# akankshabaranwal/graph-algorithm-image-segmentation-GPGPU

Hardware: NVIDIA B200
Metric: Mpixel/s end-to-end segmentation (1080p, Boruvka-Felzenszwalb, 4-connected) (higher is better)
Workload: dtype f32+u64

## Files before the change

graph-algorithm-image-segmentation-gpgpu_b200/csrc/gseg_api.cu:

```cuda
#include <cuda_runtime.h>
#include <dlfcn.h>
#include <nvjpeg.h>
#include <limits.h>
#include <stddef.h>
#include <math.h>
#include <stdio.h>
#include <stdlib.h>
#include <string.h>

#include <new>
#include <vector>

#include "../../include/gseg.h"
#include "gseg_kernels.cuh"
#include "gseg_sort.cuh"
#include "gseg_dedup.cuh"
#include "gseg_jpeg.hpp"
#include "gseg_jpeg.cuh"

#define GSEG_MAXMARK 1024
#define GRID_CAP (148 * 8)

struct GsegHead {
    GsegRunParams p;
// ... 497 lines not shown
extern "C" int gseg_input_rgb(gseg_ctx *ctx, uint8_t *out, int mem_kind) {
    if (!ctx || !out) return GSEG_E_ARG;
    if (ctx->pending) { const int rc = gseg_wait(ctx); if (rc) return rc; }
    if (!ctx->valid || !ctx->rgb_staged) return fail(ctx, GSEG_E_STATE, "the last run's input was not staged by the context", cudaSuccess);
    if (mem_kind != GSEG_MEM_HOST && mem_kind != GSEG_MEM_DEVICE) return fail(ctx, GSEG_E_ARG, "mem_kind", cudaSuccess);
    CK(cudaSetDevice(ctx->device));
    CK(cudaMemcpyAsync(out, ctx->d_rgb + (size_t)3 * ctx->w * ctx->halo_top, (size_t)3 * ctx->w * ctx->h,
                       mem_kind == GSEG_MEM_HOST ? cudaMemcpyDeviceToHost : cudaMemcpyDeviceToDevice, ctx->stream));
    CK(cudaStreamSynchronize(ctx->stream));
    return GSEG_OK;
}

extern "C" void gseg_destroy(gseg_ctx *ctx) {
    if (!ctx) return;
    cudaSetDevice(ctx->device);
    if (ctx->own_stream) cudaStreamSynchronize(ctx->own_stream);
    cudaFree(ctx->d_rgb); cudaFree(ctx->d_tmp); cudaFree(ctx->d_planes);
    cudaFree(ctx->d_G); cudaFree(ctx->d_wgrid); cudaFree(ctx->d_wsel);
    cudaFree(ctx->d_succ); cudaFree(ctx->d_rank);
    for (int i = 0; i < 2; ++i) {
        cudaFree(ctx->d_best[i]); cudaFree(ctx->d_attr[i]); cudaFree(ctx->d_csum[i]); cudaFree(ctx->d_cmean[i]);
        cudaFree(ctx->d_eab[i]); cudaFree(ctx->d_ew[i]); cudaFree(ctx->d_pcnt[i]); cudaFree(ctx->d_poff[i]); cudaFree(ctx->d_labels[i]);
    }
    cudaFree(ctx->d_pscan); cudaFree(ctx->d_arena); cudaFree(ctx->d_statusC); cudaFree(ctx->d_statusE); cudaFree(ctx->d_ctl);
    jpeg_release(ctx);
    cudaFree(ctx->d_jfile); cudaFree(ctx->d_jsamples); cudaFree(ctx->d_jdev); cudaFree(ctx->d_jcoef);
    if (ctx->h_jdesc) cudaFreeHost(ctx->h_jdesc);
    cudaFree(ctx->d_jerr); cudaFree(ctx->d_jsub);
    if (ctx->ev_jdesc) cudaEventDestroy(ctx->ev_jdesc);
    if (ctx->ev_jdone) cudaEventDestroy(ctx->ev_jdone);
    delete ctx->jplan;
    sort_scratch_free(&ctx->sort);
    cudaFree(ctx->d_xkeys); cudaFree(ctx->d_xvals); cudaFree(ctx->d_xkeep); cudaFree(ctx->d_xab); cudaFree(ctx->d_xw);
    cudaFree(ctx->d_winner); cudaFree(ctx->d_dd);
    for (int i = 0; i <= GSEG_MAXMARK; ++i)
        if (ctx->ev[i]) cudaEventDestroy(ctx->ev[i]);
    if (ctx->h_ctl) cudaFreeHost(ctx->h_ctl);
    if (ctx->h_head) cudaFreeHost(ctx->h_head);
    if (ctx->own_stream) cudaStreamDestroy(ctx->own_stream);
    free(ctx);
}

extern "C" int gseg_set_stream(gseg_ctx *ctx, void *s) {
    if (!ctx) return GSEG_E_ARG;
    if (ctx->pending) return GSEG_E_STATE;
    ctx->stream = s ? (cudaStream_t)s : ctx->own_stream;
    return GSEG_OK;
}

extern "C" int gseg_tail_cluster(const gseg_ctx *ctx) { return ctx ? ctx->tail_cluster : GSEG_E_ARG; }
extern "C" int gseg_tail_cluster_from_env(const gseg_ctx *ctx) { return ctx && ctx->tail_cluster_env ? 1 : 0; }
extern "C" void *gseg_get_stream(const gseg_ctx *ctx) { return ctx ? (void *)ctx->stream : nullptr; }

extern "C" int gseg_set_tail(gseg_ctx *ctx, uint32_t max_edges, uint32_t max_components) {
    if (!ctx) return GSEG_E_ARG;
    if (ctx->pending) return GSEG_E_STATE;
    ctx->tail_E = max_edges; ctx->tail_V = max_components;
    ctx->nbig_hint = -1;
    return GSEG_OK;
}

extern "C" int gseg_set_dedup(gseg_ctx *ctx, int on, uint32_t min_edges, uint32_t min_ratio, uint32_t max_components) {
    if (!ctx) return GSEG_E_ARG;
    if (ctx->pending) return GSEG_E_STATE;
    CK(cudaSetDevice(ctx->device));
    ctx->dd_on = on != 0;
    if (min_edges) ctx->dd_min_edges = min_edges;
    if (min_ratio) ctx->dd_min_ratio = min_ratio;
    if (max_components) ctx->dd_V = max_components;
    ctx->nbig_hint = -1; ctx->dd_skip = false;
    CK(upload_dd(ctx));
    return GSEG_OK;
}

extern "C" int gseg_set_tail_cluster(gseg_ctx *ctx, int ctas) {
    if (!ctx || ctas < 1 || ctas > 16) return GSEG_E_ARG;
    if (ctx->pending) return GSEG_E_STATE;
    CK(cudaSetDevice(ctx->device));
    ctx->tail_cluster = fit_tail_cluster(ctas);
    return GSEG_OK;
}

extern "C" int gseg_set_blocks_per_sm(gseg_ctx *ctx, int blocks) {
    if (!ctx || blocks < 1 || blocks > 8) return GSEG_E_ARG;
    if (ctx->pending) return GSEG_E_STATE;
    ctx->occ_mult = blocks;
    return GSEG_OK;
}

static int gauss_mask(float sigma, float *mask) {
    if (sigma < 0.01f) sigma = 0.01f;
    const int len = (int)ceilf(sigma * 4.0f) + 1;
    if (len > GSEG_MAXMASK) return -1;
    double m[GSEG_MAXMASK], s = 0.0;
    for (int i = 0; i < len; ++i) {
        const double t = (double)i / (double)sigma;
        m[i] = exp(-0.5 * t * t);
    }
    for (int i = 1; i < len; ++i) s += m[i];
    s = 2.0 * s + m[0];
    for (int i = 0; i < len; ++i) mask[i] = (float)(m[i] / s);
    return len;
}

static inline void mark(gseg_ctx *c, cudaStream_t s, const char *name, int round) {
    ++c->launches;
    if (!c->profiling || c->n_marks >= GSEG_MAXMARK) return;
    if (!c->ev[c->n_marks]) cudaEventCreate(&c->ev[c->n_marks]);
    cudaEventRecord(c->ev[c->n_marks], s);
    c->mark_name[c->n_marks] = name;
    c->mark_round[c->n_marks] = round;
    ++c->n_marks;
}
static inline void mark_end(gseg_ctx *c, cudaStream_t s) {
    if (!c->profiling || c->n_marks == 0 || c->n_marks >= GSEG_MAXMARK) return;
    if (!c->ev[c->n_marks]) cudaEventCreate(&c->ev[c->n_marks]);
    cudaEventRecord(c->ev[c->n_marks], s);
    c->mark_name[c->n_marks] = nullptr;
    c->mark_round[c->n_marks] = -1;
    ++c->n_marks;
}

static GsegBufs bufs_of(const gseg_ctx *c) {
    GsegBufs B;
    B.planes = c->d_planes; B.G = c->d_G; B.wgrid = c->d_wgrid;
    B.succ = c->d_succ; B.rank = c->d_rank; B.wsel = c->d_wsel; B.arena = c->d_arena;
    for (int i = 0; i < 2; ++i) {
        B.best[i] = c->d_best[i]; B.attr[i] = c->d_attr[i]; B.csum[i] = c->d_csum[i]; B.cmean[i] = c->d_cmean[i];
        B.eab[i] = c->d_eab[i]; B.ew[i] = c->d_ew[i]; B.pcnt[i] = c->d_pcnt[i]; B.poff[i] = c->d_poff[i];
    }
    B.statusC = c->d_statusC; B.statusE = c->d_statusE; B.pscan = c->d_pscan;
    return B;
}

template <int R>
static size_t blur_smem() { return (size_t)3 * (TH + 2 * R) * (BLUR_PF(R) + BLUR_PH * sizeof(float)); }
template <int R>
static void launch_blur(gseg_ctx *c, cudaStream_t s, int ntiles) {
    static bool attr[64] = {false};
    if (!attr[c->device & 63]) { cudaFuncSetAttribute(k_blur_tile<R>, cudaFuncAttributeMaxDynamicSharedMemorySize, (int)blur_smem<R>()); attr[c->device & 63] = true; }
    k_blur_tile<R><<<ntiles, NT, blur_smem<R>(), s>>>(c->d_ctl, c->d_planes);
}

template <int VARIANT, int D>
static size_t graph_smem() {
    return (size_t)(3 + D + (VARIANT == GSEG_SUPERPIX ? 1 : 0)) * BH * BW * sizeof(float) + 16;
}
template <int VARIANT, int D>
static void launch_r0_graph(gseg_ctx *c, cudaStream_t s, int ntiles, const GsegBufs &B) {
    static bool attr[64] = {false};
    if (!attr[c->device & 63]) { cudaFuncSetAttribute(k_r0_graph<VARIANT, D>, cudaFuncAttributeMaxDynamicSharedMemorySize, (int)graph_smem<VARIANT, D>()); attr[c->device & 63] = true; }
    k_r0_graph<VARIANT, D><<<ntiles < c->num_sms * c->occ_mult ? ntiles : c->num_sms * c->occ_mult, NT, graph_smem<VARIANT, D>(), s>>>(c->d_ctl, B);
}
template <int D, bool SP>
static void launch_r0_edges(gseg_ctx *c, cudaStream_t s, size_t V, const GsegBufs &B) {
    const size_t ntiles = ((size_t)D * ((V + GSEG_PAGE - 1) / GSEG_PAGE) + NT / 32 - 1) / (NT / 32);
    k_r0_edges<D, SP><<<(int)(ntiles < (size_t)c->num_sms * c->occ_mult ? ntiles : (size_t)c->num_sms * c->occ_mult), NT, 0, s>>>(c->d_ctl, B);
}

static void enqueue_round0(gseg_ctx *c, cudaStream_t s) {
    const size_t V = (size_t)c->w * c->h;
    const int variant = c->params.variant, D = c->D;
    const bool sp = variant == GSEG_SUPERPIX;
    const GsegBufs B = bufs_of(c);
    const int ntiles = ((c->w + TW - 1) / TW) * ((c->h + TH - 1) / TH);
    const int ntilesG = ((c->w + TW - 1) / TW) * ((c->h + GH - 1) / GH);
    const int R = c->h_head->p.mask_len - 1;
    if (R >= 1 && R <= 8) {
        mark(c, s, "k_blur_tile", 0);
        switch (R) {
        case 1: launch_blur<1>(c, s, ntiles); break;
        case 2: launch_blur<2>(c, s, ntiles); break;
        case 3: launch_blur<3>(c, s, ntiles); break;
        case 4: launch_blur<4>(c, s, ntiles); break;
        case 5: launch_blur<5>(c, s, ntiles); break;
        case 6: launch_blur<6>(c, s, ntiles); break;
        case 7: launch_blur<7>(c, s, ntiles); break;
        default: launch_blur<8>(c, s, ntiles); break;
        }
    } else {
        mark(c, s, "k_blur_h", 0);
        k_blur_h<<<grid_for((size_t)c->w * c->h_head->p.h_in, NT), NT, 0, s>>>(c->d_ctl, c->d_tmp);
        mark(c, s, "k_blur_v", 0);
        k_blur_v<<<grid_for(3 * V, NT), NT, 0, s>>>(c->d_ctl, c->d_tmp, c->d_planes);
    }
    if (sp) {
        mark(c, s, "k_sobel", 0);
        k_sobel<<<grid_for(V, NT), NT, 0, s>>>(c->d_ctl, c->d_planes, c->d_G);
    }
    mark(c, s, "k_r0_graph", 0);
    if (variant == GSEG_FELZ) { if (D == 2) launch_r0_graph<GSEG_FELZ, 2>(c, s, ntilesG, B); else launch_r0_graph<GSEG_FELZ, 4>(c, s, ntilesG, B); }
    else if (variant == GSEG_HIER) { if (D == 2) launch_r0_graph<GSEG_HIER, 2>(c, s, ntilesG, B); else launch_r0_graph<GSEG_HIER, 4>(c, s, ntilesG, B); }
    else { if (D == 2) launch_r0_graph<GSEG_SUPERPIX, 2>(c, s, ntilesG, B); else launch_r0_graph<GSEG_SUPERPIX, 4>(c, s, ntilesG, B); }
    mark(c, s, "k_relabel", 0);
    if (sp) k_relabel<true, true><<<grid_for(V, NT), NT, 0, s>>>(c->d_ctl, B);
    else k_relabel<true, false><<<grid_for(V, NT), NT, 0, s>>>(c->d_ctl, B);
    if (sp) {
        mark(c, s, "k_means", 0);
        k_means<<<grid_for(V, NT, c->num_sms * c->occ_mult), NT, 0, s>>>(c->d_ctl, B);
    }
    mark(c, s, "k_r0_edges", 0);
    if (D == 2) { if (sp) launch_r0_edges<2, true>(c, s, V, B); else launch_r0_edges<2, false>(c, s, V, B); }
    else { if (sp) launch_r0_edges<4, true>(c, s, V, B); else launch_r0_edges<4, false>(c, s, V, B); }
}

static void enqueue_round(gseg_ctx *c, cudaStream_t s, int r, size_t Vb, size_t Pb) {
    const bool sp = c->params.variant == GSEG_SUPERPIX;
    const GsegBufs B = bufs_of(c);
    const int cap = c->num_sms * c->occ_mult;
    if (Pb > GSEG_PSCAN_INLINE) {
        mark(c, s, "k_page_scan", r);
        k_page_scan<<<grid_for(Pb, 1024, 64), 1024, 0, s>>>(c->d_ctl, B);
    }
    mark(c, s, "k_succ_scan", r);
    if (sp) k_succ_scan<true><<<grid_for(Vb, NT * CPT, cap) + 1, NT, 0, s>>>(c->d_ctl, B);
    else k_succ_scan<false><<<grid_for(Vb, NT * CPT, cap) + 1, NT, 0, s>>>(c->d_ctl, B);
    mark(c, s, "k_relabel", r);
    if (sp) k_relabel<false, true><<<grid_for(Vb, NT, cap), NT, 0, s>>>(c->d_ctl, B);
    else k_relabel<false, false><<<grid_for(Vb, NT, cap), NT, 0, s>>>(c->d_ctl, B);
    if (sp) {
        mark(c, s, "k_means", r);
        k_means<<<grid_for(Vb, NT, cap), NT, 0, s>>>(c->d_ctl, B);
    }
    mark(c, s, "k_edges", r);
    if (sp) k_edges<true><<<grid_for(Pb, NT / 32, cap), NT, 0, s>>>(c->d_ctl, B);
    else k_edges<false><<<grid_for(Pb, NT / 32, cap), NT, 0, s>>>(c->d_ctl, B);
}

static u32 dedup_V(const gseg_ctx *c) {
    const u32 v = c->dd_V > 2u ? c->dd_V : 2u;
    return v < 65536u ? v : 65536u;
}
static bool dedup_enabled(const gseg_ctx *c) {
    return c->dd_on && c->params.variant != GSEG_SUPERPIX && !(c->params.flags & GSEG_FLAG_NO_DEDUP);
}
static bool dedup_enqueue(const gseg_ctx *c) {
    return dedup_enabled(c) &&
           !(c->dd_skip && c->hint_w == c->w && c->hint_h == c->h && c->hint_variant == c->params.variant && c->hint_conn == c->params.connectivity);
}
static void enqueue_dedup(gseg_ctx *c, cudaStream_t s, int round) {
    const GsegBufs B = bufs_of(c);
    const int cap = c->num_sms * c->occ_mult;
    const size_t ntiles = (c->dd_cap + SORT_TILE - 1) / SORT_TILE;
    const int gs = (int)(ntiles < (size_t)c->num_sms * 2 ? ntiles : (size_t)c->num_sms * 2);
    mark(c, s, "k_dd_plan", round);
    k_dd_plan<<<1, 1024, 0, s>>>(c->d_ctl, B, c->d_dd);
    mark(c, s, "k_dd_keys", round);
    k_dd_keys<<<cap, NT, 0, s>>>(c->d_ctl, B, c->d_dd);
    mark(c, s, "k_sort_scan", round);
    k_sort_scan_dev<<<4, SORT_RADIX, 0, s>>>(&c->d_dd->sort);
    for (int p = 0; p < 4; ++p) {
        mark(c, s, "k_sort_onesweep", round);
        k_sort_onesweep_dev<<<gs, SORT_NT, sort_smem_bytes(), s>>>(&c->d_dd->sort, p);
    }
    mark(c, s, "k_dd_select", round);
    k_dd_select<<<cap, NT, 0, s>>>(c->d_dd);
    mark(c, s, "k_dd_mark", round);
    k_dd_mark<<<cap, NT, 0, s>>>(c->d_ctl, B, c->d_dd);
    mark(c, s, "k_dd_compact", round);
    k_dd_compact<<<grid_for(c->dd_cap, 4096, c->num_sms * 2), 1024, 0, s>>>(c->d_ctl, B, c->d_dd);
    mark(c, s, "k_dd_finish", round);
    k_dd_finish<<<cap, NT, 0, s>>>(c->d_ctl, B, c->d_dd);
}
static bool dedup_wanted_host(const gseg_ctx *c) {
    const RoundState &st = c->h_ctl->st;
    return dedup_enabled(c) && st.phase != PH_DONE && st.round >= 1u && st.V >= 2u && st.V <= dedup_V(c) && st.E <= c->dd_cap &&
           st.E >= c->dd_min_edges && st.E / st.V >= c->dd_min_ratio;
}

static cudaError_t enqueue_tail(gseg_ctx *c, cudaStream_t s) {
    cudaLaunchConfig_t cfg = {};
    cudaLaunchAttribute at[1];
    cfg.gridDim = dim3(c->tail_cluster); cfg.blockDim = dim3(NTT);
    cfg.dynamicSmemBytes = TAIL_SMEM; cfg.stream = s;
    at[0].id = cudaLaunchAttributeClusterDimension;
    at[0].val.clusterDim.x = c->tail_cluster; at[0].val.clusterDim.y = 1; at[0].val.clusterDim.z = 1;
    cfg.attrs = at; cfg.numAttrs = 1;
    GsegCtl *ctl = c->d_ctl;
    GsegBufs B = bufs_of(c);
    mark(c, s, "k_tail", -1);
    if (c->params.variant == GSEG_SUPERPIX) return cudaLaunchKernelEx(&cfg, k_tail<true>, ctl, B);
    return cudaLaunchKernelEx(&cfg, k_tail<false>, ctl, B);
}

static size_t edge_slots(const gseg_ctx *ctx) {
    return (size_t)ctx->Dmax * ((ctx->Vmax + GSEG_PAGE - 1) / GSEG_PAGE + 1) * GSEG_PAGE;
}

static int max_rounds_of(const gseg_params *p) {
    int r = p->max_rounds > 0 ? p->max_rounds : 48;
    return r > GSEG_MAXR ? GSEG_MAXR : r;
}

static int readback(gseg_ctx *ctx) {
    CK(cudaMemcpyAsync(ctx->h_ctl, ctx->d_ctl, sizeof(GsegCtl), cudaMemcpyDeviceToHost, ctx->stream));
    CK(cudaStreamSynchronize(ctx->stream));
    return GSEG_OK;
}

static int finish(gseg_ctx *ctx) {
    ctx->pending = false;
    if (ctx->h_ctl->error == DERR_SCAN) return fail(ctx, GSEG_E_INTERNAL, "look-back watchdog", cudaSuccess);
    if (ctx->h_ctl->error == DERR_ARENA) return fail(ctx, GSEG_E_ARENA, "map arena", cudaSuccess);
    if (ctx->h_ctl->error == DERR_CHASE) return fail(ctx, GSEG_E_INTERNAL, "successor cycle", cudaSuccess);
    if (ctx->h_ctl->error == DERR_JPEG) return fail(ctx, GSEG_E_ARG, "corrupt JPEG: the entropy-coded data does not decode", cudaSuccess);
    if (ctx->h_ctl->error >= DERR_CHECK) {
        snprintf(ctx->err, sizeof(ctx->err), "checked build: bounds check at site %u failed", ctx->h_ctl->error - DERR_CHECK);
        return GSEG_E_INTERNAL;
    }
    const GsegCtl *h = ctx->h_ctl;
// ... 880 lines not shown
```

graph-algorithm-image-segmentation-gpgpu_b200/csrc/gseg_kernels.cuh:

```cuda
#pragma once
#include <cooperative_groups.h>

#include "gseg_device.cuh"

namespace cg = cooperative_groups;

#define NT 256
#ifndef GSEG_LB_SUCC
#define GSEG_LB_SUCC 4
#endif
#ifndef GSEG_LB_EDGES
#define GSEG_LB_EDGES 4
#endif
#define NTT 1024
#define CPT 4
#ifndef RUNWIN
#define RUNWIN 4
#endif

#define TW 64
#ifndef TH
#define TH 32
#endif
#define BW (TW + 4)
// ... 407 lines not shown

#define GSEG_PSCAN_INLINE 32768u
#define GSEG_TAIL_STAGE 16384u
__device__ __forceinline__ void block_scan_pages(const u32 *pcnt, u32 P, u32 *pscan, u32 *s) {
    const int lane = threadIdx.x & 31, wid = threadIdx.x >> 5, nwarp = blockDim.x >> 5;
    u32 carry = 0;
    for (u32 base = 0; base < P; base += 16u * blockDim.x) {
        const u32 i = base + 16u * threadIdx.x;
        u32 q[16];
        if (i + 15u < P) {
#pragma unroll
            for (int k = 0; k < 4; ++k) {
                const uint4 t = __ldcg(reinterpret_cast<const uint4 *>(pcnt + i) + k);
                q[4 * k] = t.x; q[4 * k + 1] = t.y; q[4 * k + 2] = t.z; q[4 * k + 3] = t.w;
            }
        } else {
#pragma unroll
            for (int k = 0; k < 16; ++k) q[k] = i + k < P ? __ldcg(pcnt + i + k) : 0u;
        }
        u32 v = 0;
#pragma unroll
        for (int k = 0; k < 16; ++k) { const u32 t = q[k]; q[k] = v; v += t; }
        const u32 inc = warp_incl_scan(v, lane);
        if (lane == 31) s[wid] = inc;
        __syncthreads();
        if (wid == 0) {
            const u32 x = lane < nwarp ? s[lane] : 0u;
            const u32 xi = warp_incl_scan(x, lane);
            s[lane] = xi - x;
            if (lane == 31) s[32] = xi;
        }
        __syncthreads();
        const u32 e = carry + s[wid] + inc - v;
        if (i + 15u < P) {
#pragma unroll
            for (int k = 0; k < 4; ++k)
                reinterpret_cast<uint4 *>(pscan + i)[k] = make_uint4(e + q[4 * k], e + q[4 * k + 1], e + q[4 * k + 2], e + q[4 * k + 3]);
        } else {
#pragma unroll
            for (int k = 0; k < 16; ++k)
                if (i + k < P) pscan[i + k] = e + q[k];
        }
        carry += s[32];
        __syncthreads();
    }
}

template <int NTH, bool R0, bool SP, bool SPREAD = false>
__device__ __forceinline__ void phase_R(const GsegCtl *ctl, const GsegBufs &B, const RoundState &st) {
    constexpr int RPT = (SPREAD || R0) ? 1 : 4;
    const int cur = st.round & 1, nxt = cur ^ 1;
    const u32 V = st.V;
    u32 *map = B.arena + st.map_off;
    const u32 V0 = (u32)ctl->p.w * (u32)ctl->p.h;
    const u32 lane = threadIdx.x & 31u, wid = threadIdx.x >> 5, nwarp = NTH / 32;
    const u32 tile0 = SPREAD ? wid * gridDim.x + blockIdx.x : blockIdx.x * nwarp + wid;
    const u32 ntile = (V + 32u * RPT - 1u) / (32u * RPT);
    for (u32 tile = tile0; tile < ntile; tile += gridDim.x * nwarp) {
        u32 c[RPT], r[RPT];
        bool act[RPT], moved[RPT];
#pragma unroll
        for (int k = 0; k < RPT; ++k) {
            c[k] = (tile * RPT + (u32)k) * 32u + lane;
            act[k] = c[k] < V;
            r[k] = act[k] ? (SPREAD ? ld_relaxed_u32(B.succ + c[k]) : B.succ[c[k]]) : c[k];
            moved[k] = r[k] != c[k];
        }
        bool busy[RPT];
#pragma unroll
        for (int k = 0; k < RPT; ++k) busy[k] = moved[k];
        for (u32 steps = 0;; ++steps) {
            u32 rr[RPT];
            bool any = false;
#pragma unroll
            for (int k = 0; k < RPT; ++k)
                if (busy[k]) rr[k] = SPREAD ? ld_relaxed_u32(B.succ + r[k]) : B.succ[r[k]];
#pragma unroll
            for (int k = 0; k < RPT; ++k)
                if (busy[k]) {
                    if (rr[k] == r[k]) busy[k] = false;
                    else { r[k] = rr[k]; any = true; }
                }
            if (!any) break;
            if (steps > V) { ((GsegCtl *)ctl)->error = DERR_CHASE; break; }
        }
        u32 m[RPT], sz[RPT], iv[RPT];
#pragma unroll
        for (int k = 0; k < RPT; ++k) {
            m[k] = 0u; sz[k] = 1u; iv[k] = 0u;
            if (act[k]) {
                GSEG_CHK(ctl, r[k] < V, 2);
                if (moved[k]) B.succ[c[k]] = r[k];
                m[k] = ld_prev<!SPREAD>(B.rank + r[k]);
                GSEG_CHK(ctl, m[k] < V && (unsigned long long)st.map_off + c[k] < ctl->p.arena_cap, 3);
            }
        }
#pragma unroll
        for (int k = 0; k < RPT; ++k)
            if (act[k]) {
                map[c[k]] = m[k];
                if (!R0) { const uint2 at = ld_prev<!SPREAD>(B.attr[cur] + c[k]); sz[k] = at.x; iv[k] = at.y; }
                if (moved[k]) iv[k] = max(iv[k], __ldcg(B.wsel + c[k]));
            }
#pragma unroll
        for (int k = 0; k < RPT; ++k) {
            warp_run_accumulate(B.attr[nxt], m[k], sz[k], iv[k], act[k]);
            if (SP && act[k]) {
                long long v0, v1, v2;
                const u32 cc = c[k];
                if (R0) { v0 = fx8(B.planes[cc]); v1 = fx8(B.planes[V0 + cc]); v2 = fx8(B.planes[2 * V0 + cc]); }
                else {
                    v0 = __ldcg(B.csum[cur] + 3 * (size_t)cc); v1 = __ldcg(B.csum[cur] + 3 * (size_t)cc + 1);
                    v2 = __ldcg(B.csum[cur] + 3 * (size_t)cc + 2);
                }
                atomicAdd((u64 *)(B.csum[nxt] + 3 * (size_t)m[k]), (u64)v0);
                atomicAdd((u64 *)(B.csum[nxt] + 3 * (size_t)m[k] + 1), (u64)v1);
                atomicAdd((u64 *)(B.csum[nxt] + 3 * (size_t)m[k] + 2), (u64)v2);
            }
        }
    }
}

template <bool SP, bool FILTER>
__device__ __forceinline__ void emit_row(const GsegBufs &B, int nxt, u32 pos, bool act, u32 a, u32 b, u32 wv,
                                         u32 fa = 0xFFFFFFFFu, u32 fb = 0xFFFFFFFFu, u32 *sfilter = nullptr) {
    u32 kb = wv;
    if (act) {
#ifndef GSEG_EXP_NOSTORE
        B.eab[nxt][pos] = make_uint2(a, b);
        B.ew[nxt][pos] = wv;
#endif
        if (SP) kb = __float_as_uint(__fmul_rn(__uint_as_float(wv), mean_dist_m(B.cmean[nxt], a, b)));
    }
#ifndef GSEG_EXP_NOMIN
    warp_run_min2<FILTER, FILTER ? 32 : RUNWIN>(B.best[nxt], a, b, kb, pos, act, fa, fb, sfilter);
#endif
}

template <bool SP>
__device__ __forceinline__ void emit_row_east(const GsegBufs &B, int nxt, u32 pos, bool act, u32 a, u32 b, u32 wv) {
    u32 kb = wv;
    if (act) {
#ifndef GSEG_EXP_NOSTORE
        B.eab[nxt][pos] = make_uint2(a, b);
        B.ew[nxt][pos] = wv;
#endif
        if (SP) kb = __float_as_uint(__fmul_rn(__uint_as_float(wv), mean_dist_m(B.cmean[nxt], a, b)));
    }
#ifndef GSEG_EXP_NOMIN
    warp_chain_min(B.best[nxt], a, b, kb, pos, act, __ballot_sync(0xFFFFFFFFu, act));
#endif
}

template <int D, bool SP>
__global__ void __launch_bounds__(NT, GSEG_LB_EDGES) k_r0_edges(GsegCtl *ctl, GsegBufs B) {
    constexpr int ROWS = GSEG_PAGE / 32;
    const int lane = threadIdx.x & 31;
    const u32 lt = (1u << lane) - 1u;
    const RoundState st = ctl->st;
    const int w = ctl->p.w, h = ctl->p.h;
    const u32 V = (u32)w * (u32)h;
    const u32 *__restrict__ map = B.arena;
    const u32 tpd = (V + GSEG_PAGE - 1) / GSEG_PAGE, ntiles = tpd * (u32)D;
    const u32 nw = gridDim.x * (NT / 32);
    u32 esum = 0;
    if (blockIdx.x == 0 && threadIdx.x == 0) ctl->ticketC = 0;
    for (u32 tile = blockIdx.x * (NT / 32) + (threadIdx.x >> 5); tile < ntiles; tile += nw) {
        const int d = (int)(tile / tpd);
        const int dx = d == 1 ? 0 : 1, dy = d == 0 ? 0 : (d == 3 ? -1 : 1);
        const int off = dy * w + dx;
        const u32 p0 = (tile - (u32)d * tpd) * GSEG_PAGE + lane;
        u32 a[ROWS], b[ROWS], m[ROWS], wv[ROWS];
        const float *wg = B.wgrid + (size_t)d * V + p0;
        int y = (int)(p0 / (u32)w), x = (int)(p0 - (u32)y * (u32)w);
#pragma unroll
        for (int j = 0; j < ROWS; ++j) {
            const u32 p = p0 + 32u * j;
            bool keep = false;
            a[j] = b[j] = wv[j] = 0u;
            if (p < V && x + dx < w && y + dy < h && y + dy >= 0) {
                a[j] = map[p];
                b[j] = map[(u32)((int)p + off)];
                wv[j] = __float_as_uint(wg[32 * j]);
                keep = a[j] != b[j];
            }
            m[j] = __ballot_sync(0xFFFFFFFFu, keep);
            x += 32;
            while (x >= w) { x -= w; ++y; }
        }
        u32 total = 0;
#pragma unroll
        for (int j = 0; j < ROWS; ++j) total += __popc(m[j]);
        if (lane == 0) { B.pcnt[1][tile] = total; B.poff[1][tile] = tile * GSEG_PAGE; }
        GSEG_CHK(ctl, (unsigned long long)tile * GSEG_PAGE + total <= ctl->p.edge_slots, 4);
        esum += total;
        u32 rowoff = tile * GSEG_PAGE;
#pragma unroll
        for (int j = 0; j < ROWS; ++j) {
            if (m[j] == 0u) continue;
            const bool act = (m[j] >> lane) & 1u;
            if (d == 0) emit_row_east<SP>(B, 1, rowoff + __popc(m[j] & lt), act, a[j], b[j], wv[j]);
            else emit_row<SP, false>(B, 1, rowoff + __popc(m[j] & lt), act, a[j], b[j], wv[j]);
            rowoff += __popc(m[j]);
        }
    }
    if (lane == 0 && esum) atomicAdd(&ctl->Eacc[0], esum);
    RoundState s0 = st;
    s0.P = ntiles;
    last_block_advance(ctl, s0, 1u);
}

template <bool SP, bool SPREAD>
__device__ __forceinline__ void phase_S(GsegCtl *ctl, const GsegBufs &B, const RoundState &st, u32 *sh) {
    constexpr u32 TILE_C = 32 * CPT;
    const int lane = threadIdx.x & 31, wid = threadIdx.x >> 5, nwarp = blockDim.x >> 5;
    const u32 lt = (1u << lane) - 1u;
    const int cur = st.round & 1, nxt = cur ^ 1;
    const u32 V = st.V;
    const u32 nwt = (V + TILE_C - 1) / TILE_C;
    const u32 ntiles = (nwt + nwarp - 1) / nwarp;
    const u32 tag = ctl->p.epoch_base + st.round * 2u + 1u;
    const u64 *best = B.best[cur];
    const uint2 *eab = B.eab[cur], *attr = B.attr[cur];
    const float kk = ctl->p.k;
    const u32 min_size = (u32)ctl->p.min_size, phase = st.phase;
    const bool pred = ctl->p.variant == GSEG_FELZ && phase == PH_PRED;
    const bool msz = ctl->p.variant == GSEG_FELZ && phase == PH_MINSIZE;
    if (blockIdx.x == 0 && threadIdx.x == 0) ctl->ticketE = 0;
    u32 stile = (u32)wid * gridDim.x + blockIdx.x;
    auto write_ids = [&](u32 pre, u32 base, const u32 *m, u32 total) {
        u32 rowoff = pre;
#pragma unroll
        for (int j = 0; j < CPT; ++j) {
            if ((m[j] >> lane) & 1u) B.rank[base + 32u * j] = rowoff + __popc(m[j] & lt);
            rowoff += __popc(m[j]);
        }
        for (u32 i = lane; i < total; i += 32u) {
            const u32 n = pre + i;
            B.attr[nxt][n] = make_uint2(0u, 0u); B.best[nxt][n] = GSEG_KEY_NONE;
            if (SP) { B.csum[nxt][3 * (size_t)n] = 0; B.csum[nxt][3 * (size_t)n + 1] = 0; B.csum[nxt][3 * (size_t)n + 2] = 0; }
        }
    };
    auto finish_block = [&](u32 btile, u32 base, u32 below, u32 all, const u32 *m, u32 total) {
        if (wid == 0) {
            const u32 pre = lookback_resolve(B.statusC, btile, tag, all, &ctl->error);
            if (lane == 0) sh[64] = pre;
        }
        __syncthreads();
        const u32 bpre = sh[64];
        if (btile == ntiles - 1 && threadIdx.x == 0) ctl->Vnext = bpre + all;
        write_ids(bpre + below, base, m, total);
        __syncthreads();
    };
    bool p_have = false;
    u32 p_btile = 0, p_base = 0, p_below = 0, p_all = 0, p_total = 0, p_m[CPT] = {};
    for (;;) {
        u32 btile = 0, tile;
        if (SPREAD) {
            tile = stile;
            if (tile >= nwt) break;
            stile += gridDim.x * (u32)nwarp;
        } else {
            if (threadIdx.x == 0) sh[65] = atomicAdd(&ctl->ticketC, 1u);
            __syncthreads();
            btile = sh[65];
            if (btile >= ntiles) break;
            tile = btile * nwarp + wid;
        }
        const u32 base = tile * TILE_C + lane;
        u64 key[CPT], key2[CPT];
        uint2 ab[CPT], ta[CPT], tb[CPT];
#pragma unroll
        for (int j = 0; j < CPT; ++j) key[j] = base + 32u * j < V ? ld_prev<!SPREAD>(best + base + 32u * j) : GSEG_KEY_NONE;
#pragma unroll
        for (int j = 0; j < CPT; ++j) {
            GSEG_CHK(ctl, key[j] == GSEG_KEY_NONE || (u32)key[j] < ctl->p.edge_slots, 5);
            ab[j] = key[j] != GSEG_KEY_NONE ? ld_prev<!SPREAD>(eab + (u32)key[j]) : make_uint2(0u, 0u);
        }
#pragma unroll
        for (int j = 0; j < CPT; ++j) {
            key2[j] = GSEG_KEY_NONE; ta[j] = tb[j] = make_uint2(1u, 0u);
            if (key[j] != GSEG_KEY_NONE) {
                const u32 c = base + 32u * j, other = ab[j].x == c ? ab[j].y : ab[j].x;
                GSEG_CHK(ctl, (ab[j].x == c || ab[j].y == c) && other < V && other != c, 6);
                key2[j] = ld_prev<!SPREAD>(best + other);
                if (pred || msz) { ta[j] = ld_prev<!SPREAD>(attr + ab[j].x); tb[j] = ld_prev<!SPREAD>(attr + ab[j].y); }
            }
        }
        u32 m[CPT], total = 0;
#pragma unroll
        for (int j = 0; j < CPT; ++j) {
            const u32 c = base + 32u * j;
            bool root = false;
            if (c < V) {
                u32 s = c, wb = 0u;
                if (key[j] != GSEG_KEY_NONE) {
                    wb = (u32)(key[j] >> 32);
                    const bool c_is_a = ab[j].x == c;
                    const u32 other = c_is_a ? ab[j].y : ab[j].x;
                    bool ok = true, other_ok = true;
                    if (pred) {
                        const float wt = __uint_as_float(wb);
                        const float fa = __fadd_rn(__uint_as_float(ta[j].y), __fdiv_rn(kk, __uint2float_rn(ta[j].x)));
                        const float fb = __fadd_rn(__uint_as_float(tb[j].y), __fdiv_rn(kk, __uint2float_rn(tb[j].x)));
                        ok = wt <= fa && wt <= fb;
                    } else if (msz) {
                        ok = (c_is_a ? ta[j].x : tb[j].x) < min_size;
                        other_ok = (c_is_a ? tb[j].x : ta[j].x) < min_size;
                    }
                    if (ok) {
                        s = other;
                        if (key2[j] == key[j] && other_ok && c < other) s = c;
                    }
                }
                B.succ[c] = s;
                B.wsel[c] = wb;
                root = s == c;
            }
            m[j] = __ballot_sync(0xFFFFFFFFu, root);
            total += __popc(m[j]);
        }
        if (SPREAD) {
            const u32 pre = lookback_prefix(B.statusC, tile, tag, total, &ctl->error);
            if (tile == nwt - 1 && lane == 0) ctl->Vnext = pre + total;
            write_ids(pre, base, m, total);
        } else {
            if (lane == 0) sh[wid] = total;
            __syncthreads();
            const u32 v = lane < nwarp ? sh[lane] : 0u;
            u32 below = lane < wid ? v : 0u, all = v;
#pragma unroll
            for (int o = 16; o; o >>= 1) { below += __shfl_xor_sync(0xFFFFFFFFu, below, o); all += __shfl_xor_sync(0xFFFFFFFFu, all, o); }
            if (wid == 0) lookback_publish(B.statusC, btile, tag, all);
            __syncthreads();
            if (p_have) finish_block(p_btile, p_base, p_below, p_all, p_m, p_total);
            p_have = true; p_btile = btile; p_base = base; p_below = below; p_all = all; p_total = total;
#pragma unroll
            for (int j = 0; j < CPT; ++j) p_m[j] = m[j];
        }
    }
    if (!SPREAD && p_have) finish_block(p_btile, p_base, p_below, p_all, p_m, p_total);
}

template <bool SP, bool SPREAD, int RW>
__device__ __forceinline__ void phase_E_rows(GsegCtl *ctl, const GsegBufs &B, const RoundState &st, u32 Vnext, u32 *stage) {
    constexpr int ROWS = GSEG_PAGE / 32;
    const int lane = threadIdx.x & 31;
    const u32 lt = (1u << lane) - 1u;
    const int cur = st.round & 1, nxt = cur ^ 1;
    const u32 E = st.E, P = st.P;
    const uint2 *eab = B.eab[cur];
    const u32 *ew = B.ew[cur];
    const u32 *pc = B.pcnt[cur], *po = B.poff[cur];
    const u32 *map = B.arena + st.map_off;
    const bool filter = (E >> ctl->p.filter_shift) > Vnext;
    const u32 G = group_size(st), ngroups = (P + G - 1u) / G;
    if (blockIdx.x == 0 && threadIdx.x == 0) ctl->ticketC = 0;
// ... 458 lines not shown
```

Before: 9685.

## Stage round-0 edge inputs via double-buffered TMA bulk copies per warp

Adds a staged variant of k_r0_edges in which each warp prefetches its next page's label, neighbour-label and weight streams into shared memory with cp.async.bulk and mbarriers, double-buffered, so global loads overlap with compaction and emission of the current page. The host picks the staged variant when pages per warp stay under a threshold and otherwise falls back to the original direct-load path. The staged path needs about 50KB of dynamic shared memory per block, which may lower occupancy, and it adds per-page barrier waits.

Measured after the change: 10060, median of 6. +3.9%, better.

```diff
diff --git a/graph-algorithm-image-segmentation-gpgpu_b200/csrc/gseg_api.cu b/graph-algorithm-image-segmentation-gpgpu_b200/csrc/gseg_api.cu
--- a/graph-algorithm-image-segmentation-gpgpu_b200/csrc/gseg_api.cu
+++ b/graph-algorithm-image-segmentation-gpgpu_b200/csrc/gseg_api.cu
@@ -673,10 +673,16 @@
     if (!attr[c->device & 63]) { cudaFuncSetAttribute(k_r0_graph<VARIANT, D>, cudaFuncAttributeMaxDynamicSharedMemorySize, (int)graph_smem<VARIANT, D>()); attr[c->device & 63] = true; }
     k_r0_graph<VARIANT, D><<<ntiles < c->num_sms * c->occ_mult ? ntiles : c->num_sms * c->occ_mult, NT, graph_smem<VARIANT, D>(), s>>>(c->d_ctl, B);
 }
+#define R0_STAGE_MAX_PPW 128
 template <int D, bool SP>
 static void launch_r0_edges(gseg_ctx *c, cudaStream_t s, size_t V, const GsegBufs &B) {
-    const size_t ntiles = ((size_t)D * ((V + GSEG_PAGE - 1) / GSEG_PAGE) + NT / 32 - 1) / (NT / 32);
-    k_r0_edges<D, SP><<<(int)(ntiles < (size_t)c->num_sms * c->occ_mult ? ntiles : (size_t)c->num_sms * c->occ_mult), NT, 0, s>>>(c->d_ctl, B);
+    static bool attr[64] = {false};
+    if (!attr[c->device & 63]) { cudaFuncSetAttribute(k_r0_edges<D, SP, true>, cudaFuncAttributeMaxDynamicSharedMemorySize, (int)R0_SMEM); attr[c->device & 63] = true; }
+    const size_t pages = (size_t)D * ((V + GSEG_PAGE - 1) / GSEG_PAGE);
+    const size_t ntiles = (pages + NT / 32 - 1) / (NT / 32);
+    const int grid = (int)(ntiles < (size_t)c->num_sms * c->occ_mult ? ntiles : (size_t)c->num_sms * c->occ_mult);
+    if (pages <= (size_t)R0_STAGE_MAX_PPW * grid * (NT / 32)) k_r0_edges<D, SP, true><<<grid, NT, R0_SMEM, s>>>(c->d_ctl, B);
+    else k_r0_edges<D, SP, false><<<grid, NT, 0, s>>>(c->d_ctl, B);
 }
 
 static void enqueue_round0(gseg_ctx *c, cudaStream_t s) {
diff --git a/graph-algorithm-image-segmentation-gpgpu_b200/csrc/gseg_kernels.cuh b/graph-algorithm-image-segmentation-gpgpu_b200/csrc/gseg_kernels.cuh
--- a/graph-algorithm-image-segmentation-gpgpu_b200/csrc/gseg_kernels.cuh
+++ b/graph-algorithm-image-segmentation-gpgpu_b200/csrc/gseg_kernels.cuh
@@ -583,37 +583,144 @@
 #endif
 }
 
-template <int D, bool SP>
+__device__ __forceinline__ u32 smem_addr(const void *p) { return (u32)__cvta_generic_to_shared(p); }
+__device__ __forceinline__ void mbar_init(u64 *bar) {
+    asm volatile("mbarrier.init.shared::cta.b64 [%0], 1;\n\tfence.mbarrier_init.release.cluster;" ::"r"(smem_addr(bar)) : "memory");
+}
+__device__ __forceinline__ void mbar_expect_tx(u64 *bar, u32 bytes) {
+    asm volatile("mbarrier.arrive.expect_tx.shared::cta.b64 _, [%0], %1;" ::"r"(smem_addr(bar)), "r"(bytes) : "memory");
+}
+__device__ __forceinline__ void mbar_wait(u64 *bar, u32 parity) {
+    asm volatile("{\n\t.reg .pred P1;\n\tWAIT:\n\t"
+                 "mbarrier.try_wait.parity.shared::cta.b64 P1, [%0], %1;\n\t"
+                 "@!P1 bra WAIT;\n\t}" ::"r"(smem_addr(bar)), "r"(parity) : "memory");
+}
+__device__ __forceinline__ void bulk_copy(void *dst, const void *src, u32 bytes, u64 *bar) {
+    asm volatile("cp.async.bulk.shared::cluster.global.mbarrier::complete_tx::bytes [%0], [%1], %2, [%3];"
+                 ::"r"(smem_addr(dst)), "l"(src), "r"(bytes), "r"(smem_addr(bar)) : "memory");
+}
+__device__ __forceinline__ void fence_proxy_async() { asm volatile("fence.proxy.async.shared::cta;" ::: "memory"); }
+
+#define R0_STREAM 264
+#define R0_BUF (3 * R0_STREAM)
+#define R0_SMEM ((NT / 32) * (2 * R0_BUF * 4 + 16))
+struct R0Page {
+    int d, off;
+    u32 p0;
+    u32 src[3];
+    u32 n[3];
+};
+__device__ __forceinline__ R0Page r0_page(u32 tile, u32 tpd, u32 V, int w) {
+    R0Page pg;
+    pg.d = (int)(tile / tpd);
+    pg.off = pg.d == 0 ? 1 : pg.d == 1 ? w : pg.d == 2 ? w + 1 : 1 - w;
+    pg.p0 = (tile - (u32)pg.d * tpd) * GSEG_PAGE;
+    const long long end = min((long long)pg.p0 + GSEG_PAGE, (long long)V);
+    const long long lo[3] = {pg.p0, max((long long)pg.p0 + pg.off, 0LL), (long long)pg.d * V + pg.p0};
+    const long long hi[3] = {end, min(end + pg.off, (long long)V), (long long)pg.d * V + end};
+#pragma unroll
+    for (int s = 0; s < 3; ++s) {
+        pg.src[s] = (u32)(lo[s] & ~3LL);
+        pg.n[s] = hi[s] > lo[s] ? (u32)(((hi[s] + 3) & ~3LL) - (lo[s] & ~3LL)) : 0u;
+    }
+    return pg;
+}
+
+template <int D, bool SP, bool STAGED>
 __global__ void __launch_bounds__(NT, GSEG_LB_EDGES) k_r0_edges(GsegCtl *ctl, GsegBufs B) {
     constexpr int ROWS = GSEG_PAGE / 32;
-    const int lane = threadIdx.x & 31;
+    extern __shared__ __align__(16) u32 r0_stage[];
+    const int lane = threadIdx.x & 31, wid = threadIdx.x >> 5;
     const u32 lt = (1u << lane) - 1u;
     const RoundState st = ctl->st;
     const int w = ctl->p.w, h = ctl->p.h;
     const u32 V = (u32)w * (u32)h;
     const u32 *__restrict__ map = B.arena;
+    const u32 *__restrict__ wgrid = reinterpret_cast<const u32 *>(B.wgrid);
     const u32 tpd = (V + GSEG_PAGE - 1) / GSEG_PAGE, ntiles = tpd * (u32)D;
     const u32 nw = gridDim.x * (NT / 32);
+    u64 *bar = reinterpret_cast<u64 *>(r0_stage) + 2 * wid;
+    u32 *buf = r0_stage + 4 * (NT / 32) + wid * 2 * R0_BUF;
+    auto stage = [&](u32 tile, u32 k) {
+        const R0Page pg = r0_page(tile, tpd, V, w);
+        u32 *dst = buf + k * R0_BUF;
+        fence_proxy_async();
+        mbar_expect_tx(bar + k, 4u * (pg.n[0] + pg.n[1] + pg.n[2]));
+        bulk_copy(dst, map + pg.src[0], 4u * pg.n[0], bar + k);
+        if (pg.n[1]) bulk_copy(dst + R0_STREAM, map + pg.src[1], 4u * pg.n[1], bar + k);
+        bulk_copy(dst + 2 * R0_STREAM, wgrid + pg.src[2], 4u * pg.n[2], bar + k);
+    };
     u32 esum = 0;
     if (blockIdx.x == 0 && threadIdx.x == 0) ctl->ticketC = 0;
-    for (u32 tile = blockIdx.x * (NT / 32) + (threadIdx.x >> 5); tile < ntiles; tile += nw) {
-        const int d = (int)(tile / tpd);
+    u32 tile = blockIdx.x * (NT / 32) + wid;
+    if constexpr (!STAGED) {
+        for (; tile < ntiles; tile += nw) {
+            const int d = (int)(tile / tpd);
+            const int dx = d == 1 ? 0 : 1, dy = d == 0 ? 0 : (d == 3 ? -1 : 1);
+            const int off = dy * w + dx;
+            const u32 p0 = (tile - (u32)d * tpd) * GSEG_PAGE + lane;
+            u32 a[ROWS], b[ROWS], m[ROWS], wv[ROWS];
+            const u32 *wg = wgrid + (size_t)d * V + p0;
+            int y = (int)(p0 / (u32)w), x = (int)(p0 - (u32)y * (u32)w);
+#pragma unroll
+            for (int j = 0; j < ROWS; ++j) {
+                const u32 p = p0 + 32u * j;
+                bool keep = false;
+                a[j] = b[j] = wv[j] = 0u;
+                if (p < V && x + dx < w && y + dy < h && y + dy >= 0) {
+                    a[j] = map[p];
+                    b[j] = map[(u32)((int)p + off)];
+                    wv[j] = wg[32 * j];
+                    keep = a[j] != b[j];
+                }
+                m[j] = __ballot_sync(0xFFFFFFFFu, keep);
+                x += 32;
+                while (x >= w) { x -= w; ++y; }
+            }
+            u32 total = 0;
+#pragma unroll
+            for (int j = 0; j < ROWS; ++j) total += __popc(m[j]);
+            if (lane == 0) { B.pcnt[1][tile] = total; B.poff[1][tile] = tile * GSEG_PAGE; }
+            GSEG_CHK(ctl, (unsigned long long)tile * GSEG_PAGE + total <= ctl->p.edge_slots, 4);
+            esum += total;
+            u32 rowoff = tile * GSEG_PAGE;
+#pragma unroll
+            for (int j = 0; j < ROWS; ++j) {
+                if (m[j] == 0u) continue;
+                const bool act = (m[j] >> lane) & 1u;
+                if (d == 0) emit_row_east<SP>(B, 1, rowoff + __popc(m[j] & lt), act, a[j], b[j], wv[j]);
+                else emit_row<SP, false>(B, 1, rowoff + __popc(m[j] & lt), act, a[j], b[j], wv[j]);
+                rowoff += __popc(m[j]);
+            }
+        }
+    } else {
+    if (lane == 0) {
+        mbar_init(bar);
+        mbar_init(bar + 1);
+        if (tile < ntiles) stage(tile, 0u);
+    }
+    __syncwarp();
+    for (u32 it = 0; tile < ntiles; tile += nw, ++it) {
+        const u32 k = it & 1u;
+        __syncwarp();
+        if (lane == 0 && tile + nw < ntiles) stage(tile + nw, k ^ 1u);
+        const R0Page pg = r0_page(tile, tpd, V, w);
+        const int d = pg.d, off = pg.off;
         const int dx = d == 1 ? 0 : 1, dy = d == 0 ? 0 : (d == 3 ? -1 : 1);
-        const int off = dy * w + dx;
-        const u32 p0 = (tile - (u32)d * tpd) * GSEG_PAGE + lane;
-        u32 a[ROWS], b[ROWS], m[ROWS], wv[ROWS];
-        const float *wg = B.wgrid + (size_t)d * V + p0;
+        const u32 p0 = pg.p0 + lane;
+        const u32 *sa = buf + k * R0_BUF + lane;
+        const u32 *sb = buf + k * R0_BUF + R0_STREAM + (int)(pg.p0 + off - pg.src[1]) + lane;
+        const u32 *sw = buf + k * R0_BUF + 2 * R0_STREAM + (d * V + pg.p0 - pg.src[2]) + lane;
+        u32 m[ROWS], live = 0u;
         int y = (int)(p0 / (u32)w), x = (int)(p0 - (u32)y * (u32)w);
+        mbar_wait(bar + k, (it >> 1) & 1u);
 #pragma unroll
         for (int j = 0; j < ROWS; ++j) {
             const u32 p = p0 + 32u * j;
             bool keep = false;
-            a[j] = b[j] = wv[j] = 0u;
             if (p < V && x + dx < w && y + dy < h && y + dy >= 0) {
-                a[j] = map[p];
-                b[j] = map[(u32)((int)p + off)];
-                wv[j] = __float_as_uint(wg[32 * j]);
-                keep = a[j] != b[j];
+                live |= 1u << j;
+                keep = sa[32 * j] != sb[32 * j];
             }
             m[j] = __ballot_sync(0xFFFFFFFFu, keep);
             x += 32;
@@ -629,11 +736,13 @@
 #pragma unroll
         for (int j = 0; j < ROWS; ++j) {
             if (m[j] == 0u) continue;
-            const bool act = (m[j] >> lane) & 1u;
-            if (d == 0) emit_row_east<SP>(B, 1, rowoff + __popc(m[j] & lt), act, a[j], b[j], wv[j]);
-            else emit_row<SP, false>(B, 1, rowoff + __popc(m[j] & lt), act, a[j], b[j], wv[j]);
+            const bool act = (m[j] >> lane) & 1u, in = (live >> j) & 1u;
+            const u32 a = in ? sa[32 * j] : 0u, b = in ? sb[32 * j] : 0u, wv = in ? sw[32 * j] : 0u;
+            if (d == 0) emit_row_east<SP>(B, 1, rowoff + __popc(m[j] & lt), act, a, b, wv);
+            else emit_row<SP, false>(B, 1, rowoff + __popc(m[j] & lt), act, a, b, wv);
             rowoff += __popc(m[j]);
         }
+    }
     }
     if (lane == 0 && esum) atomicAdd(&ctl->Eacc[0], esum);
     RoundState s0 = st;
```
